# apache/paimon

Measured on NVIDIA H100. Metric: merged rows/sec at 16 runs x 40M rows, higher is better.
Workload: dtype int64

## Files before the change

### paimon_b200/csrc/parquet_decode.cu

```cuda
#include <algorithm>
#include <cstring>
#include <memory>
#include <stdexcept>

#include "device_utils.cuh"
#include "parquet_meta.h"
#include "inflate_device.cuh"
#include "scan_kernels.cuh"
#include "zstd_device.cuh"

namespace pg {

enum : int { ENC_PLAIN = 0, ENC_DICT = 1, ENC_DELTA_BP = 2, ENC_RLE_BOOL = 3 };

struct PqChunk {
    const uint8_t *base;
    int64_t avail;
    int64_t num_values;
    int64_t row0;
    int32_t col, run, file, codec;
    int32_t max_def, phys, phys_width;
    int32_t cast;
    int32_t n_pages, n_dicts;
    int64_t scratch_bytes;
// ... 794 lines not shown
                s_vs[warp][lane][c] = (int32_t)(p + bias);
                bias -= 4;
                p += 4 + len;
                if (++j == nnz) break;
            }
            if (bad || j == nnz) done = true;
        }
        __syncwarp();
        for (unsigned m = __ballot_sync(0xffffffffu, j > j0); m != 0; m &= m - 1) {
            const int i = __ffs(m) - 1;
            const int n = __shfl_sync(0xffffffffu, j - j0, i);
            int32_t *dst = (int32_t *)__shfl_sync(0xffffffffu, (unsigned long long)(uintptr_t)(vs + j0), i);
            if (lane < n) dst[lane] = s_vs[warp][i][lane];
        }
        WT_MARK(2);
        if (__all_sync(0xffffffffu, done)) break;
        const int cur = (int)(p / kWvChunk);
        const int first = max(next, cur);
        const int nreq = done ? 0 : max(0, min(min(cur, hist[0]) + kWvRing, n_chunks) - first);
        next = first + nreq;
        int incl = nreq;
#pragma unroll
        for (int d = 1; d < 32; d <<= 1) {
            const int y = __shfl_up_sync(0xffffffffu, incl, d);
            if (lane >= d) incl += y;
        }
        const int total = __shfl_sync(0xffffffffu, incl, 31);
        for (int r = 0; r < nreq; r++) {
            const int k = first + r;
            const uint32_t units = min(8u, (pend - (uint32_t)k * kWvChunk + 15) / 16);
            s_req_src[warp][incl - nreq + r] = a0 + (size_t)k * kWvChunk;
            s_req_dst[warp][incl - nreq + r] = (uint32_t)lane << 8 | (uint32_t)(k % kWvRing) << 4 | units;
        }
        __syncwarp();
        for (int e = lane >> 3; e < total; e += 4) {
            const uint32_t d = s_req_dst[warp][e], u = lane & 7;
            if (u < (d & 15)) {
                const int owner = (int)(d >> 8), unit = (int)(((d >> 4) & 15) * 8 + u);
                cp_async16(&rows[owner][(unit ^ (owner & 15)) << 4], s_req_src[warp][e] + 16 * u);
            }
        }
        cp_async_commit();
#pragma unroll
        for (int i = 0; i < kWvLead; i++) hist[i] = hist[i + 1];
        hist[kWvLead] = next;
        WT_MARK(0);
    }
    cp_async_wait<0>();
    WT_END(nnz);
    if (mine) {
        if (bad || (nnz > 0 && p != pend) || (nnz == 0 && slen != 0)) { pq_err(err, KERR_BAD_PAGE); pages[t].bad = 1; return; }
        vs[nnz] = (int32_t)(p + bias);
    }
}

constexpr int kExpThreads = 256;
constexpr int kPayIn = 8 * 1024, kPayOut = 7 * 1024;
constexpr int kPayBatches = 1023;


__device__ __forceinline__ uint64_t pq_load_unaligned(const uint8_t *p, int w) {
    if (w == 8) {
        const uintptr_t a = (uintptr_t)p;
        const uint64_t *q = (const uint64_t *)(a & ~(uintptr_t)7);
        const int sh = (int)(a & 7) * 8;
        const uint64_t lo = q[0];
        return sh ? (lo >> sh) | (q[1] << (64 - sh)) : lo;
    }
    const uintptr_t a = (uintptr_t)p;
    const uint32_t *q = (const uint32_t *)(a & ~(uintptr_t)3);
    const int sh = (int)(a & 3) * 8;
    const uint32_t lo = q[0];
    return sh ? (uint64_t)((lo >> sh) | (q[1] << (32 - sh))) : (uint64_t)lo;
}

template <bool kPlainStrings> struct PqPlainStage {
    int vs[2][kExpThreads + 4];
    int bnd[kPayBatches + 1];
    alignas(16) uint8_t in[2][kPayIn];
    alignas(16) uint8_t out[kPayOut];
};
template <> struct PqPlainStage<false> {};

template <bool kPlainStrings>
__global__ void __launch_bounds__(kExpThreads, 6)
k_pq_expand(const PqPage *pages, const PqPage *dicts, const PqChunk *chunks, const PqOut *outs, int n_cols,
            const int32_t *ids, const int32_t *vstart, const int32_t *dict_off, const int32_t *dict_len) {
    __shared__ uint32_t s_bits[kExpThreads];
    __shared__ int s_rank[kExpThreads];
    __shared__ int s_wlen[kExpThreads];
    __shared__ int s_ws[34];
    __shared__ PqPlainStage<kPlainStrings> stage;
    const PqPage pg = pages[blockIdx.x];
    if (pg.bad || pg.num_values == 0) return;
    const PqChunk ch = chunks[pg.chunk];
    if (kPlainStrings != (ch.phys == pq::T_BYTE_ARRAY && pg.enc == ENC_PLAIN)) return;
    const PqOut out = outs[ch.run * n_cols + ch.col];
    const int tid = threadIdx.x, lane = tid & 31, warp = tid >> 5;
    const int64_t row0 = pg.row0, row1 = pg.row0 + pg.num_values;
    const int64_t g0 = row0 & ~(int64_t)31;
    const int n_words = (int)((row1 - g0 + 31) >> 5);
    const uint8_t *values = pg.body + pg.values_off;
    const int pw = ch.phys_width;
    const bool varlen = ch.phys == pq::T_BYTE_ARRAY;
    const bool is_dict = pg.enc == ENC_DICT;
    const PqPage *dj = is_dict ? &dicts[ch.dict_base] : nullptr;
    const uint8_t *dbody = is_dict ? dj->body : nullptr;
    const int64_t ebase = is_dict ? dj->entry_base : 0;
    const int32_t *pids = ids + pg.ids_base;
    const int32_t *vs = vstart + pg.vs_base;
    uint8_t *payload = varlen ? (uint8_t *)out.data : nullptr;
    int carry_rank = 0;
    int64_t carry_bytes = pg.payload_base;
    for (int w0 = 0; w0 < n_words; w0 += kExpThreads) {
        const int jw = w0 + tid;
        uint32_t bits = 0;
        if (jw < n_words) {
            const int64_t wrow = g0 + 32 * (int64_t)jw;
            const int lo = wrow < row0 ? (int)(row0 - wrow) : 0;
            const int64_t hi = pq_min64(32, row1 - wrow);
            const uint32_t mask = (hi >= 32 ? 0xffffffffu : ((1u << hi) - 1)) & ~((1u << lo) - 1);
            bits = out.validity ? (out.validity[wrow >> 5] & mask) : mask;
        }
        int tot = 0;
        const int excl = block_scan_excl(__popc(bits), s_ws, &tot);
        s_bits[tid] = bits;
        s_rank[tid] = carry_rank + excl;
        __syncthreads();
        const int nw = min(kExpThreads, n_words - w0);
        if (varlen && is_dict) {
            for (int jj = warp; jj < nw; jj += kExpThreads / 32) {
                const uint32_t b = s_bits[jj];
                int len = 0;
                if ((b >> lane) & 1) len = dict_len[ebase + pids[s_rank[jj] + __popc(b & ((1u << lane) - 1))]];
#pragma unroll
                for (int d = 16; d > 0; d >>= 1) len += __shfl_xor_sync(0xffffffffu, len, d);
                if (lane == 0) s_wlen[jj] = len;
            }
            __syncthreads();
            int wtot = 0;
            const int wl = tid < nw ? s_wlen[tid] : 0;
            const int wex = block_scan_excl(wl, s_ws, &wtot);
            s_wlen[tid] = wex;
            __syncthreads();
            for (int jj = warp; jj < nw; jj += kExpThreads / 32) {
                const uint32_t b = s_bits[jj];
                const int64_t row = g0 + 32 * (int64_t)(w0 + jj) + lane;
                const bool inpage = row >= row0 && row < row1;
                int len = 0;
                const uint8_t *src = nullptr;
                if ((b >> lane) & 1) {
                    const int id = pids[s_rank[jj] + __popc(b & ((1u << lane) - 1))];
                    len = dict_len[ebase + id];
                    src = dbody + dict_off[ebase + id];
                }
                const int incl = warp_scan_incl(len);
                const int64_t off = carry_bytes + s_wlen[jj] + incl - len;
                if (inpage) out.offsets[row] = (int32_t)off;
                for (int r8 = 0; r8 < 32; r8 += 4) {
                    const int sl = r8 + (lane >> 3);
                    const int64_t o2 = __shfl_sync(0xffffffffu, off, sl);
                    const int l2 = __shfl_sync(0xffffffffu, len, sl);
                    const uint8_t *s2 = (const uint8_t *)__shfl_sync(0xffffffffu, (unsigned long long)(uintptr_t)src, sl);
                    for (int bb = lane & 7; bb < l2; bb += 8) payload[o2 + bb] = s2[bb];
                }
            }
            carry_bytes += wtot;
        } else {
            constexpr int kExpUnroll = 4, kStep = kExpThreads / 32;
            const int fmode = varlen ? 0 : pg.enc == ENC_RLE_BOOL ? 1 : ch.phys == pq::T_BOOLEAN ? 2 : is_dict ? 3 : 4;
            if (fmode == 4 && pw == 8 && out.out_width == 8 && ch.cast == 0) {
                constexpr int kPairUnroll = 2;
                const int half = lane >> 4, p0 = 2 * (lane & 15);
                const uintptr_t a0 = (uintptr_t)values;
                const int sh = (int)(a0 & 7) * 8;
                const uint64_t *q0 = (const uint64_t *)(a0 & ~(uintptr_t)7);
                uint64_t *od = (uint64_t *)out.data;
                for (int j0 = 2 * warp; j0 < nw; j0 += 2 * kStep * kPairUnroll) {
                    int64_t row[kPairUnroll];
// ... 100 lines not shown
        }
        carry_rank += tot;
        __syncthreads();
    }
    if (varlen) {
        if constexpr (kPlainStrings) {
            auto &s_vs = stage.vs;
            auto &s_bnd = stage.bnd;
            auto &s_in = stage.in;
            auto &s_out = stage.out;
            const int nnz = pg.nnz;
            const int64_t pb = pg.payload_base;
            const int nb = (nnz + kExpThreads - 1) / kExpThreads;
            const bool staged_page = nb <= kPayBatches;
            __syncthreads();
            if (staged_page) for (int i = tid; i <= nb; i += kExpThreads) s_bnd[i] = vs[min(i * kExpThreads, nnz)];
            __syncthreads();
            auto batch_src = [&](int b2) -> const uint8_t * { return values + ((int64_t)s_bnd[b2] - pb) + 4 * (int64_t)b2 * kExpThreads; };
            auto batch_fits = [&](int b2) -> bool {
                const int jn = min(kExpThreads, nnz - b2 * kExpThreads);
                const int out_len = s_bnd[b2 + 1] - s_bnd[b2];
                const int iskew = (int)((uintptr_t)batch_src(b2) & 15), oskew = (int)((uintptr_t)(payload + s_bnd[b2]) & 15);
                return iskew + out_len + 4 * jn <= kPayIn && oskew + out_len <= kPayOut;
            };
            auto prefetch = [&](int b2) {
                const int jn = min(kExpThreads, nnz - b2 * kExpThreads);
                int *dv = s_vs[b2 & 1];
                for (int i = tid; i <= jn; i += kExpThreads) cp_async4(dv + i, vs + b2 * kExpThreads + i);
                if (batch_fits(b2)) {
                    const uint8_t *src0 = batch_src(b2);
                    const int iskew = (int)((uintptr_t)src0 & 15);
                    const int n16 = (iskew + (s_bnd[b2 + 1] - s_bnd[b2]) + 4 * jn + 15) >> 4;
                    uint8_t *di = s_in[b2 & 1];
                    for (int i = tid; i < n16; i += kExpThreads) cp_async16(di + 16 * i, src0 - iskew + 16 * i);
                }
                cp_async_commit();
            };
            if (staged_page && nb > 0) prefetch(0);
            for (int b2 = 0; b2 < nb; b2++) {
                const int j0 = b2 * kExpThreads, jn = min(kExpThreads, nnz - j0);
                if (!staged_page) {
                    for (int t = tid >> 3; t < jn; t += kExpThreads / 8) {
                        const int st = vs[j0 + t], len = vs[j0 + t + 1] - st;
                        const uint8_t *src = values + ((int64_t)st - pb) + 4 * (int64_t)(j0 + t + 1);
                        for (int b3 = tid & 7; b3 < len; b3 += 8) payload[(int64_t)st + b3] = src[b3];
                    }
                    continue;
                }
                if (b2 + 1 < nb) { prefetch(b2 + 1); cp_async_wait<1>(); } else cp_async_wait<0>();
                __syncthreads();
                const int *cvs = s_vs[b2 & 1];
                const int out0 = s_bnd[b2], out_len = s_bnd[b2 + 1] - out0;
                if (batch_fits(b2)) {
                    const uint8_t *src0 = batch_src(b2);
                    const int iskew = (int)((uintptr_t)src0 & 15), oskew = (int)((uintptr_t)(payload + out0) & 15);
                    if (tid < jn) {
                        const int o = cvs[tid] - out0, len = cvs[tid + 1] - cvs[tid];
                        const uint8_t *sp = s_in[b2 & 1] + iskew + o + 4 * (tid + 1);
                        uint8_t *dp = s_out + oskew + o;
                        for (int b3 = 0; b3 < len; b3++) dp[b3] = sp[b3];
                    }
                    __syncthreads();
                    uint8_t *dst16 = payload + out0 - oskew;
                    const int end = oskew + out_len;
                    for (int c = tid; c * 16 < end; c += kExpThreads) {
                        const int c0 = c * 16;
                        if (c0 >= oskew && c0 + 16 <= end) *(uint4 *)(dst16 + c0) = *(const uint4 *)(s_out + c0);
                        else for (int b3 = max(c0, oskew); b3 < min(c0 + 16, end); b3++) dst16[b3] = s_out[b3];
                    }
                } else {
                    for (int t = tid >> 3; t < jn; t += kExpThreads / 8) {
                        const int st = cvs[t], len = cvs[t + 1] - st;
                        const uint8_t *src = values + ((int64_t)st - pb) + 4 * (int64_t)(j0 + t + 1);
                        for (int b3 = tid & 7; b3 < len; b3 += 8) payload[(int64_t)st + b3] = src[b3];
                    }
                }
                __syncthreads();
            }
        }
        if (pg.is_last && tid == 0) out.offsets[row1] = (int32_t)(pg.payload_base + pg.payload_bytes);
    }
}

__global__ void k_pq_zero_first_offset(const PqOut *outs, int n) {
    const int i = blockIdx.x * blockDim.x + threadIdx.x;
    if (i < n && outs[i].offsets) outs[i].offsets[0] = 0;
}


static int phys_cast(int pg_t, int phys) {
    switch (pg_t) {
        case PG_INT8: case PG_INT16: case PG_INT32: return phys == pq::T_INT32 ? 0 : -1;
        case PG_INT64: return phys == pq::T_INT64 ? 0 : (phys == pq::T_INT32 ? 1 : -1);
        case PG_FLOAT: return phys == pq::T_FLOAT ? 0 : -1;
        case PG_DOUBLE: return phys == pq::T_DOUBLE ? 0 : (phys == pq::T_FLOAT ? 2 : -1);
        case PG_BOOL: return phys == pq::T_BOOLEAN ? 0 : -1;
        case PG_STRING: case PG_BINARY: return phys == pq::T_BYTE_ARRAY ? 0 : -1;
        default: return -1;
    }
}
static int phys_width_of(int phys) {
    return phys == pq::T_INT32 || phys == pq::T_FLOAT ? 4 : (phys == pq::T_INT64 || phys == pq::T_DOUBLE ? 8 : 0);
}

static pg_status map_file_schema(RunBuilder &b, const pq::FileMetaData &m, int run) {
    if (m.schema.empty()) return fail(PG_ERR_FORMAT, "parquet: empty schema");
    const int nleaf = (int)m.schema.size() - 1;
    if (m.schema[0].num_children != nleaf)
        return fail(PG_ERR_UNSUPPORTED, "parquet: nested columns are not decoded on device (flat KeyValue file schemas are)");
    std::vector<std::string> cols(nleaf);
    for (int i = 1; i <= nleaf; i++) {
        if (m.schema[i].num_children != 0 || m.schema[i].repetition == pq::R_REPEATED)
            return fail(PG_ERR_UNSUPPORTED, "parquet: nested / repeated column " + m.schema[i].name);
        cols[i - 1] = m.schema[i].name;
    }
    { pg_status st = b.add_file(run, m.num_rows, cols); if (st) return st; }
    for (int c = 0; c < b.nc; c++) {
        const int fc = b.file_col.back()[c];
        if (fc < 0) continue;
        const pq::SchemaElement &e = m.schema[fc + 1];
        if (phys_cast(b.schema->field(c).type, e.type) < 0)
            return fail(PG_ERR_UNSUPPORTED, "parquet: column " + e.name + " has a physical type the device decoder "
                                            "does not map to the table type");
    }
    for (const pq::RowGroup &g : m.row_groups) {
        if ((int)g.columns.size() != nleaf) return fail(PG_ERR_FORMAT, "parquet: row group with a different column count");
        for (const pq::ColumnChunk &cc : g.columns)
            if (cc.codec != pq::C_UNCOMPRESSED && cc.codec != pq::C_SNAPPY && cc.codec != pq::C_ZSTD && cc.codec != pq::C_GZIP)
                return fail(PG_ERR_UNSUPPORTED, "parquet: compression codec " + std::to_string(cc.codec) +
                                                " is not decoded on device (UNCOMPRESSED, SNAPPY, ZSTD and GZIP are); write with "
                                                "'file.compression'='zstd' / 'snappy' / 'gzip' / 'none' or let the Java side decompress");
    }
    return PG_OK;
}

static pg_status kernel_error_status(int code) {
    switch (code) {
        case KERR_NONE: return PG_OK;
        case KERR_PQ_ENCODING:
            return fail(PG_ERR_UNSUPPORTED, "parquet: a page uses a value encoding the device decoder does not implement "
                                            "(PLAIN, dictionary, DELTA_BINARY_PACKED integers and RLE booleans are decoded)");
        case KERR_PQ_LEVELS:
            return fail(PG_ERR_UNSUPPORTED, "parquet: repetition levels / BIT_PACKED definition levels are not decoded on device");
        case KERR_PQ_NO_DICT: return fail(PG_ERR_FORMAT, "parquet: dictionary-encoded page without dictionary");
        case KERR_PQ_ROWS: return fail(PG_ERR_FORMAT, "parquet: page row counts do not add up");
        case KERR_PQ_HEADER: return fail(PG_ERR_FORMAT, "parquet: malformed or truncated page header");
        case KERR_PQ_DICT_ID: return fail(PG_ERR_FORMAT, "parquet: dictionary id outside the dictionary");
        case KERR_OFFSET_OVERFLOW: return fail(PG_ERR_INTERNAL, "parquet: a var-len column exceeds 2 GiB of payload");
        default: return fail(PG_ERR_FORMAT, "parquet: a page does not expand to its declared size");
    }
}

struct SectionFile {
    const uint8_t *bytes;
    int64_t size;
    int mem;
    int run;
    const pq::FileMetaData *meta;
};

static pg_status fetch_footers(const std::vector<SectionFile> &files, cudaStream_t sm, std::vector<pq::FileMetaData> &own_meta,
                               std::vector<const pq::FileMetaData *> &meta) {
    const int nf = (int)files.size();
    std::vector<int> need;
    for (int f = 0; f < nf; f++) {
        if (files[f].meta) meta[f] = files[f].meta;
        else if (files[f].mem == PG_MEM_DEVICE) need.push_back(f);
    }
    std::vector<uint8_t> tails(8 * need.size() + 8);
    SmallReads rb(sm);
    for (size_t i = 0; i < need.size(); i++) {
        pg_status rs = rb.add(tails.data() + 8 * i, files[need[i]].bytes + files[need[i]].size - 8, 8);
        if (rs) return rs;
    }
    if (!need.empty()) { pg_status rs = rb.finish(); if (rs) return rs; }
    std::vector<std::vector<uint8_t>> footers(need.size());
    try {
        for (size_t i = 0; i < need.size(); i++) {
            const int64_t flen = pq::footer_length(tails.data() + 8 * i);
            if (flen + 12 > files[need[i]].size) return fail(PG_ERR_FORMAT, "parquet: bad footer length");
            footers[i].resize((size_t)flen + 8);
            pg_status rs = rb.add(footers[i].data(), files[need[i]].bytes + files[need[i]].size - 8 - flen, (size_t)flen);
            if (rs) return rs;
        }
        if (!need.empty()) { pg_status rs = rb.finish(); if (rs) return rs; }
        for (size_t i = 0; i < need.size(); i++) {
            own_meta[need[i]] = pq::parse_footer_thrift(footers[i].data(), (int64_t)footers[i].size() - 8);
            meta[need[i]] = &own_meta[need[i]];
        }
        for (int f = 0; f < nf; f++)
            if (!meta[f]) {
                own_meta[f] = pq::parse_footer(files[f].bytes, files[f].size);
                meta[f] = &own_meta[f];
            }
    } catch (const std::exception &e) {
        return fail(PG_ERR_FORMAT, e.what());
    }
    return PG_OK;
}

struct ChunkTables {
    std::vector<PqChunk> chunks;
    std::vector<PqPair> pairs;
    bool any_snappy = false, any_delta = false, any_zstd = false;
    int64_t pair_rows = 0;
};

static pg_status build_chunk_tables(const Schema *s, const std::vector<SectionFile> &files,
                                    const std::vector<const uint8_t *> &d_file, const std::vector<const pq::FileMetaData *> &meta,
                                    const RunBuilder &b, ChunkTables &t) {
    const int nc = s->n_cols();
    const int n_runs = (int)b.run_rows.size();
    std::vector<std::vector<int>> run_files(n_runs);
    for (int f = 0; f < (int)files.size(); f++) run_files[files[f].run].push_back(f);
    for (int r = 0; r < n_runs; r++) {
        for (int c = 0; c < nc; c++) {
            if (!b.read[c]) continue;
            const int chunk0 = (int)t.chunks.size();
            for (int f : run_files[r]) {
                const pq::FileMetaData &m = *meta[f];
                const int fc = b.file_col[f][c];
                int64_t rg_row0 = 0;
                int64_t rows = 0;
                if (fc < 0) continue;
                for (const pq::RowGroup &g : m.row_groups) {
                    const pq::ColumnChunk &cc = g.columns[fc];
                    const int64_t start = cc.start();
                    if (cc.num_values != g.num_rows) return fail(PG_ERR_FORMAT, "parquet: page row counts do not add up");
                    if (cc.num_values == 0) continue;
                    if (start < 4 || start >= files[f].size) return fail(PG_ERR_FORMAT, "parquet: page offset out of range");
                    PqChunk ch;
                    memset(&ch, 0, sizeof(ch));
                    ch.base = d_file[f] + start;
                    ch.avail = std::min<int64_t>(cc.total_compressed_size > 0 ? cc.total_compressed_size : files[f].size,
                                                 files[f].size - start);
                    ch.num_values = cc.num_values;
                    ch.row0 = b.file_row0[f] + rg_row0;
                    ch.col = c; ch.run = r; ch.file = f; ch.codec = cc.codec;
                    ch.max_def = m.schema[fc + 1].repetition == pq::R_OPTIONAL ? 1 : 0;
                    ch.phys = cc.type;
                    ch.phys_width = phys_width_of(cc.type);
                    ch.cast = phys_cast(s->field(c).type, cc.type);
                    if (cc.type != m.schema[fc + 1].type) return fail(PG_ERR_FORMAT, "parquet: column chunk type differs from the schema");
                    if (cc.codec == pq::C_SNAPPY) t.any_snappy = true;
                    if (cc.codec == pq::C_ZSTD || cc.codec == pq::C_GZIP) t.any_zstd = true;
                    for (int32_t e : cc.encodings) if (e == pq::E_DELTA_BINARY_PACKED) t.any_delta = true;
                    if (cc.num_values > 0) t.chunks.push_back(ch);
                    rg_row0 += g.num_rows;
                    rows += g.num_rows;
                }
                if (rows != m.num_rows) return fail(PG_ERR_FORMAT, "parquet: row group row counts do not add up");
            }
            if (is_varlen(s->field(c).type)) {
                PqPair pr{r, c, chunk0, (int)t.chunks.size(), t.pair_rows, (int)t.pairs.size(), 0};
                t.pairs.push_back(pr);
                t.pair_rows += b.run_rows[r];
            }
        }
    }
    return PG_OK;
}

#ifdef PG_WALK_TIMING
static void walk_timing_dump() {
    static long long h[kWtSlots][8];
    cudaDeviceSynchronize();
    cudaMemcpyFromSymbol(h, g_walk_ts, sizeof(h));
    double acc[3] = {0, 0, 0}, steps = 0, vals = 0, steps_max = 0;
    long long g_lo = LLONG_MAX, g_hi = 0;
    int n = 0;
    for (int s = 0; s < kWtSlots; s++) {
        if (h[s][4] == 0) continue;
        n++;
        for (int k = 0; k < 3; k++) acc[k] += (double)h[s][k];
        steps += (double)h[s][3];
        steps_max = std::max(steps_max, (double)h[s][3]);
        vals += (double)h[s][4];
        g_lo = std::min(g_lo, h[s][5]);
        g_hi = std::max(g_hi, h[s][6]);
    }
    if (n == 0) return;
    const double tot = acc[0] + acc[1] + acc[2];
    fprintf(stderr, "[walk timing] %d warps: cycles per step issue %.0f wait %.0f walk %.0f (%.1f / %.1f / %.1f %%); "
                    "steps per warp %.1f (max %.0f), values per lane-step %.2f, span %.3f ms\n",
            n, acc[0] / steps, acc[1] / steps, acc[2] / steps, 100 * acc[0] / tot, 100 * acc[1] / tot, 100 * acc[2] / tot,
            steps / n, steps_max, vals / (32.0 * steps), (g_hi - g_lo) * 1e-6);
    int hist[10] = {0};
    double busy = 0;
    for (int s = 0; s < kWtSlots; s++) {
        if (h[s][4] == 0) continue;
        hist[std::min(9, (int)(10.0 * (h[s][5] - g_lo) / (double)(g_hi - g_lo + 1)))]++;
        busy += (double)(h[s][6] - h[s][5]);
    }
    fprintf(stderr, "[walk timing] warp start by tenth of the span:");
    for (int i = 0; i < 10; i++) fprintf(stderr, " %d", hist[i]);
    fprintf(stderr, "; mean warp lifetime %.3f ms\n", busy / n * 1e-6);
    static long long z[kWtSlots][8];
    cudaMemcpyToSymbol(g_walk_ts, z, sizeof(z));
}
#endif

static pg_status expand_pages(cudaStream_t sm, bool byte_arrays, PqPage *d_pages, int np, const PqPage *d_dicts,
                              const PqChunk *d_chunks, const PqOut *d_outs, int nc, const int32_t *d_ids, int32_t *d_vstart,
                              const int32_t *d_dict_off, const int32_t *d_dict_len, int32_t *d_err, int *launches) {
    if (!byte_arrays) {
        k_pq_expand<false><<<np, kExpThreads, 0, sm>>>(d_pages, d_dicts, d_chunks, d_outs, nc, d_ids, d_vstart,
                                                       d_dict_off, d_dict_len);
        (*launches)++;
        return PG_OK;
    }
    static thread_local cudaStream_t side = nullptr;
    static thread_local cudaEvent_t ev_fork = nullptr, ev_join = nullptr;
    if (!side) {
        int prio_lo = 0, prio_hi = 0;
        cudaDeviceGetStreamPriorityRange(&prio_lo, &prio_hi);
        PG_CUDA(cudaStreamCreateWithPriority(&side, cudaStreamNonBlocking, prio_hi));
        PG_CUDA(cudaEventCreateWithFlags(&ev_fork, cudaEventDisableTiming));
        PG_CUDA(cudaEventCreateWithFlags(&ev_join, cudaEventDisableTiming));
    }
    PG_CUDA(cudaEventRecord(ev_fork, sm));
    PG_CUDA(cudaStreamWaitEvent(side, ev_fork, 0));
    k_pq_walk_values<<<(np + kWvWarps * 32 - 1) / (kWvWarps * 32), kWvWarps * 32, 0, side>>>(
        d_pages, np, d_chunks, d_vstart, d_err);
    k_pq_expand<true><<<np, kExpThreads, 0, side>>>(d_pages, d_dicts, d_chunks, d_outs, nc, d_ids, d_vstart, d_dict_off,
                                                    d_dict_len);
    PG_CUDA(cudaEventRecord(ev_join, side));
    k_pq_expand<false><<<np, kExpThreads, 0, sm>>>(d_pages, d_dicts, d_chunks, d_outs, nc, d_ids, d_vstart, d_dict_off,
                                                   d_dict_len);
    PG_CUDA(cudaStreamWaitEvent(sm, ev_join, 0));
#ifdef PG_WALK_TIMING
    walk_timing_dump();
#endif
    *launches += 3;
    return PG_OK;
}

static pg_status decode_section(const std::shared_ptr<const Schema> &s, const std::vector<SectionFile> &files,
                                int n_runs, const char *const *names, const uint8_t *read_cols, uint64_t *out_runs,
                                pg_section_info *info) {
    const int nc = s->n_cols();
    const int nf = (int)files.size();
    cudaStream_t sm = copy_stream();
    Scratch scratch(sm);
    RunBuilder b(s, n_runs, scratch, "parquet");
    int launches = 0;
    SectionTimer tm;
    PG_CUDA(cudaEventCreate(&tm.e0));
    PG_CUDA(cudaEventCreate(&tm.e1));
    { pg_status st = b.read_columns(read_cols, names); if (st) return st; }

    std::vector<const uint8_t *> d_file(nf, nullptr);
    std::vector<pq::FileMetaData> own_meta(nf);
    std::vector<const pq::FileMetaData *> meta(nf, nullptr);
    int64_t file_bytes = 0, h2d = 0;
    PG_CUDA(cudaEventRecord(tm.e0, sm));
    for (int f = 0; f < nf; f++) {
        const SectionFile &sf = files[f];
        if (sf.size < 12) return fail(PG_ERR_FORMAT, "parquet: missing PAR1 magic (encrypted or not a Parquet file)");
        file_bytes += sf.size;
        if (sf.mem == PG_MEM_DEVICE) d_file[f] = sf.bytes;
        else {
            { pg_status st = file_image(scratch, sf.bytes, sf.size, "parquet", &d_file[f]); if (st) return st; }
            h2d += sf.size;
        }
    }
    { pg_status st = fetch_footers(files, sm, own_meta, meta); if (st) return st; }
    std::vector<uint8_t> any_optional(nc, 0);
    for (int f = 0; f < nf; f++) {
        pg_status st = map_file_schema(b, *meta[f], files[f].run);
        if (st) return st;
        for (int c = 0; c < nc; c++) {
            const int fc = b.file_col[f][c];
            if (fc == -1 || (fc >= 0 && meta[f]->schema[fc + 1].repetition == pq::R_OPTIONAL)) any_optional[c] = 1;
        }
    }
    { pg_status st = b.check_runs(); if (st) return st; }
    ChunkTables ct;
    { pg_status st = build_chunk_tables(s.get(), files, d_file, meta, b, ct); if (st) return st; }
    const int n_chunks = (int)ct.chunks.size(), n_pairs = (int)ct.pairs.size();

    { pg_status st = b.alloc(any_optional, b.missing); if (st) return st; }
    std::vector<PqOut> outs((size_t)n_runs * nc);
    auto fill_outs = [&] {
        for (size_t i = 0; i < outs.size(); i++) {
            const int t = s->field((int)(i % nc)).type;
            outs[i] = PqOut{b.out[i].data, b.out[i].offsets, b.out[i].validity, type_width(t), t == PG_BOOL};
        }
    };
    fill_outs();
    const bool any_empty = std::find(b.run_rows.begin(), b.run_rows.end(), 0) != b.run_rows.end();

    const size_t tb_chunks = align256(sizeof(PqChunk) * (size_t)std::max(n_chunks, 1));
    const size_t tb_outs = align256(sizeof(PqOut) * outs.size());
    const size_t tb_pairs = align256(sizeof(PqPair) * (size_t)std::max(n_pairs, 1));
    const size_t tb_tot = align256(sizeof(int64_t) * (size_t)(8 + n_pairs));
    unsigned char *tb = (unsigned char *)scratch.take(tb_chunks + tb_outs + tb_pairs + tb_tot + 256);
    if (!tb) return oom("parquet", "the chunk tables", tb_chunks + tb_outs + tb_pairs + tb_tot);
    PqChunk *d_chunks = (PqChunk *)tb;
    PqOut *d_outs = (PqOut *)(tb + tb_chunks);
    PqPair *d_pairs = (PqPair *)(tb + tb_chunks + tb_outs);
    int64_t *d_totals = (int64_t *)(tb + tb_chunks + tb_outs + tb_pairs);
    int32_t *d_err = (int32_t *)(d_totals + 6);
    PG_CUDA(cudaMemsetAsync(d_totals, 0, tb_tot, sm));
    if (n_chunks) { pg_status ts = small_h2d(d_chunks, ct.chunks.data(), sizeof(PqChunk) * n_chunks, sm); if (ts) return ts; }
    { pg_status ts = small_h2d(d_outs, outs.data(), sizeof(PqOut) * outs.size(), sm); if (ts) return ts; }
    if (n_pairs) { pg_status ts = small_h2d(d_pairs, ct.pairs.data(), sizeof(PqPair) * n_pairs, sm); if (ts) return ts; }
    int64_t h_tot[8] = {0, 0, 0, 0, 0, 0, 0, 0};
    if (n_chunks) {
        k_pq_walk<false><<<(n_chunks + 63) / 64, 64, 0, sm>>>(d_chunks, n_chunks, nullptr, nullptr, nullptr, d_err);
        k_pq_chunk_scan<<<1, kScanThreads, 0, sm>>>(d_chunks, n_chunks, d_totals);
        launches += 2;
// ... 3 lines not shown
            if (!rs) rs = rb.finish();
            if (rs) return rs;
        }
        const int herr = (int)(h_tot[6] & 0xffffffff);
        if (herr != KERR_NONE) return kernel_error_status(herr);
    }
    const int64_t n_pages = h_tot[0], n_dicts = h_tot[1], sc_bytes = h_tot[2], dict_entries = h_tot[3],
                  ids_entries = h_tot[4], page_bytes = h_tot[5];
    if (n_pages > 0x7fffffffLL) return fail(PG_ERR_UNSUPPORTED, "parquet: too many pages in one section");

    const size_t sb_pages = align256(sizeof(PqPage) * (size_t)std::max<int64_t>(n_pages, 1));
    const size_t sb_dicts = align256(sizeof(PqPage) * (size_t)std::max<int64_t>(n_dicts, 1));
    const size_t sb_sc = align256((size_t)sc_bytes + 64);
    const size_t sb_de = align256(4 * (size_t)(dict_entries + 1));
    const size_t sb_ids = align256(4 * (size_t)(ids_entries + 1));
    const size_t sb_vs = align256(4 * (size_t)(ct.pair_rows + n_pages + n_pairs + 2));
    int zs_ctas = 0;
    if (ct.any_zstd) {
        int dev = 0, sms = 132;
        cudaGetDevice(&dev);
        cudaDeviceGetAttribute(&sms, cudaDevAttrMultiProcessorCount, dev);
        zs_ctas = (int)std::min<int64_t>((int64_t)sms * 5, (n_pages + n_dicts + kZsWarps - 1) / kZsWarps);
    }
    const size_t sb_zs = align256((size_t)zs_ctas * kZsWarps * (size_t)(zs::kMaxBlock + 64));
    unsigned char *sbuf = (unsigned char *)scratch.take(sb_pages + sb_dicts + sb_sc + 2 * sb_de + sb_ids + sb_vs + sb_zs + 256);
    if (!sbuf) return oom("parquet", "the page table and scratch", sb_pages + sb_dicts + sb_sc + 2 * sb_de + sb_ids + sb_vs + sb_zs);
    PqPage *d_pages = (PqPage *)sbuf;
    PqPage *d_dicts = (PqPage *)(sbuf + sb_pages);
    uint8_t *d_sc = sbuf + sb_pages + sb_dicts;
    int32_t *d_dict_off = (int32_t *)(d_sc + sb_sc);
    int32_t *d_dict_len = (int32_t *)(d_sc + sb_sc + sb_de);
    int32_t *d_ids = (int32_t *)(d_sc + sb_sc + 2 * sb_de);
    int32_t *d_vstart = (int32_t *)(d_sc + sb_sc + 2 * sb_de + sb_ids);
    uint8_t *d_zs_lit = (uint8_t *)d_vstart + sb_vs;
    const int np = (int)n_pages, nd = (int)n_dicts;
    std::vector<int64_t> pair_tot(std::max(n_pairs, 1), 0);
    if (np > 0) {
        k_pq_walk<true><<<(n_chunks + 63) / 64, 64, 0, sm>>>(d_chunks, n_chunks, d_pages, d_dicts, d_sc, d_err);
        launches++;
        if (ct.any_snappy) {
            const int64_t th = (int64_t)(np + nd) * 32;
            k_pq_snappy<<<(unsigned)((th + 127) / 128), 128, 0, sm>>>(d_pages, np, d_dicts, nd, d_chunks, d_err);
            launches++;
        }
        if (ct.any_zstd && zs_ctas > 0) {
            k_pq_zstd<<<zs_ctas, kZsWarps * 32, 0, sm>>>(d_pages, np, d_dicts, nd, d_chunks, d_zs_lit, (int32_t *)(d_totals + 7), d_err);
            launches++;
        }
        if (ct.any_delta) {
            k_pq_delta<<<(unsigned)(((int64_t)np * 32 + 127) / 128), 128, 0, sm>>>(d_pages, np, d_chunks, d_err);
            launches++;
        }
        if (dict_entries > 0) {
            k_pq_walk_dicts<<<(nd + kWalkWarps - 1) / kWalkWarps, kWalkWarps * 32, 0, sm>>>(
                d_dicts, nd, d_chunks, d_dict_off, d_dict_len, d_err);
            launches++;
        }
        k_pq_levels<<<(unsigned)(((int64_t)np * 32 + 127) / 128), 128, 0, sm>>>(d_pages, np, d_dicts, d_chunks, d_outs, nc,
                                                                            d_ids, d_dict_len, d_err);
        launches++;
        if (n_pairs) {
            k_pq_scan_pages<<<(n_pairs * 32 + 127) / 128, 128, 0, sm>>>(d_pages, d_chunks, d_pairs, n_pairs, d_totals + 8, d_err);
            launches++;
            {
                SmallReads rb(sm);
                pg_status rs = rb.add(pair_tot.data(), d_totals + 8, sizeof(int64_t) * n_pairs);
                if (!rs) rs = rb.add(h_tot, d_totals, sizeof(int64_t) * 8);
                if (!rs) rs = rb.finish();
                if (rs) return rs;
            }
            const int herr = (int)(h_tot[6] & 0xffffffff);
            if (herr != KERR_NONE) return kernel_error_status(herr);
        }
    }

    if (n_pairs) {
        std::vector<int64_t> payload((size_t)n_runs * nc, 0);
        for (const PqPair &pr : ct.pairs) payload[(size_t)pr.run * nc + pr.col] = pair_tot[pr.idx];
        { pg_status st = b.alloc_payload(payload); if (st) return st; }
        fill_outs();
        { pg_status ts = small_h2d(d_outs, outs.data(), sizeof(PqOut) * outs.size(), sm); if (ts) return ts; }
    }
    if (np > 0) {
        pg_status st = expand_pages(sm, n_pairs > 0, d_pages, np, d_dicts, d_chunks, d_outs, nc, d_ids, d_vstart, d_dict_off,
                                    d_dict_len, d_err, &launches);
        if (st) return st;
    }
    if (any_empty && n_pairs) {
        k_pq_zero_first_offset<<<(n_runs * nc + 127) / 128, 128, 0, sm>>>(d_outs, n_runs * nc);
        launches++;
    }
    PG_CUDA(cudaEventRecord(tm.e1, sm));
    {
        SmallReads rb(sm);
        pg_status rs = rb.add(h_tot, d_totals, sizeof(int64_t) * 8);
        if (!rs) rs = rb.finish();
        if (rs) return rs;
    }
    PG_CUDA(cudaGetLastError());
    {
        const int herr = (int)(h_tot[6] & 0xffffffff);
        if (herr != KERR_NONE) return kernel_error_status(herr);
    }
    b.finish(out_runs, h2d, info);
    if (info) {
        info->file_bytes = file_bytes;
        info->page_bytes = page_bytes;
        info->n_files = nf;
        info->n_chunks = n_chunks;
        info->n_data_pages = np;
        info->n_dictionary_pages = nd;
        info->launches = launches;
        info->ms_decode = tm.ms();
    }
    return PG_OK;
}


struct PqReader {
    std::shared_ptr<const Schema> schema;
    pq::FileMetaData meta;
    std::vector<uint8_t> file;
    int64_t n_rows = 0;
    int n_data_pages = 0, n_dict_pages = 0;
    float ms_decode = 0;
    int launches = 0;
};

static Table<PqReader> g_pq(5);

static pg_status pq_open(uint64_t schema, const uint8_t *bytes, int64_t size, uint64_t *out) {
    std::shared_ptr<Schema> s = g_schemas.get(schema);
    if (!s || !bytes || !out) return fail(PG_ERR_INVALID, "bad schema handle or null argument");
    auto rd = std::make_unique<PqReader>();
    rd->schema = s;
    try {
        rd->meta = pq::parse_footer(bytes, size);
    } catch (const std::exception &e) {
        return fail(PG_ERR_FORMAT, e.what());
    }
    const pq::FileMetaData &m = rd->meta;
    Scratch scratch(nullptr);
    RunBuilder b(s, 1, scratch, "parquet");
    pg_status st = map_file_schema(b, m, 0);
    if (st) return st;
    const int nc = s->n_cols();
    rd->n_rows = m.num_rows;
    int64_t row0 = 0;
    for (const pq::RowGroup &g : m.row_groups) {
        for (int c = 0; c < nc; c++) {
            const pq::ColumnChunk &cc = g.columns[c];
            const int max_def = m.schema[c + 1].repetition == pq::R_OPTIONAL ? 1 : 0;
            int64_t pos = cc.start(), vals = 0;
            bool have_dict = false;
            while (vals < cc.num_values) {
                if (pos < 4 || pos >= size) return fail(PG_ERR_FORMAT, "parquet: page offset out of range");
                PqHeader h;
                if (!pq_parse_header(bytes + pos, bytes + size, h)) return fail(PG_ERR_FORMAT, "parquet: malformed or truncated page header");
                const int64_t body = pos + h.hdr;
                if (h.comp < 0 || body + h.comp > size) return fail(PG_ERR_FORMAT, "parquet: truncated page");
                if (h.type == pq::P_DICTIONARY) {
                    if (h.enc != pq::E_PLAIN && h.enc != pq::E_PLAIN_DICTIONARY)
                        return fail(PG_ERR_UNSUPPORTED, "parquet: dictionary page encoding");
                    have_dict = true;
                    rd->n_dict_pages++;
                } else if (h.type == pq::P_DATA || h.type == pq::P_DATA_V2) {
                    const bool is_dict = h.enc == pq::E_PLAIN_DICTIONARY || h.enc == pq::E_RLE_DICTIONARY;
                    const bool is_delta = h.enc == pq::E_DELTA_BINARY_PACKED && (cc.type == pq::T_INT32 || cc.type == pq::T_INT64);
// ... 202 lines not shown
```

### profiles/decode_kernels.py

```python
import argparse
import collections
import json
import os
import subprocess
import sys
import tempfile

ROOT = os.path.dirname(os.path.dirname(os.path.abspath(__file__)))
sys.path.insert(0, ROOT)
os.environ.setdefault("PG_RUN_CACHE_BYTES", str(64 << 30))


def gpu_identity(index):
    try:
        out = subprocess.run(["nvidia-smi", "-i", str(index), "--query-gpu=name,power.limit,clocks.max.sm",
                              "--format=csv,noheader"], capture_output=True, text=True, timeout=30).stdout.strip()
        name, power, clock = [x.strip() for x in out.split(",")]
        return {"name": name, "power_limit": power, "clocks_max_sm": clock}
    except Exception as e:
        import torch
        return {"name": torch.cuda.get_device_name(index), "power_limit": None, "error": repr(e)[:200]}


def decode_windows(kernels):
    wins, cur = [], []
    for k in kernels:
        if "k_pq_walk<false>" in k["name"] and cur:
            wins.append(cur)
            cur = []
        cur.append(k)
    if cur:
        wins.append(cur)
    return wins


def short(name):
    n = name.split("(")[0]
    return n.replace("pg::", "").replace("void ", "")


def main():
    ap = argparse.ArgumentParser()
    ap.add_argument("--rows", type=int, default=None, help="total input rows (default: the bench's C3 size)")
    ap.add_argument("--reps", type=int, default=3)
    ap.add_argument("--warmup", type=int, default=2)
    ap.add_argument("--out", default=os.path.join(tempfile.gettempdir(), "decode_kernels"))
    args = ap.parse_args()

    import torch
    from torch.profiler import ProfilerActivity, profile

    import bench
    from paimon_b200 import _native as N
    from paimon_b200.format import read_section

    dev = torch.device("cuda", 0)
    torch.cuda.set_device(dev)
    w = bench.WORKLOADS["c3"]
    rows = args.rows or w["rows"]
    schema = bench.make_schema("c3")
    lib = N.init(0)
    _, images, _, _ = bench.device_parquet_files("c3", schema, rows, dev, 100, lib)
    files = [(img, r) for r, img in enumerate(images)]

    def decode():
        readers, info = read_section(schema, files, w["n_runs"], 0)
        for r in readers:
            r.close()
        return info

    for _ in range(args.warmup):
        decode()
    torch.cuda.synchronize()
    infos = []
    with profile(activities=[ProfilerActivity.CUDA]) as prof:
        for _ in range(args.reps):
            infos.append(decode())
        torch.cuda.synchronize()
    os.makedirs(args.out, exist_ok=True)
    trace = os.path.join(args.out, "trace.pt.trace.json")
    prof.export_chrome_trace(trace)
    with open(trace) as f:
        ev = json.load(f)["traceEvents"]
    kernels = sorted(({"name": e["name"], "ts": float(e["ts"]), "dur": float(e["dur"]),
                       "stream": e.get("args", {}).get("stream")}
                      for e in ev if e.get("cat") == "kernel" and "k_pq" in e.get("name", "")),
                     key=lambda k: k["ts"])
    wins = decode_windows(kernels)
    n = len(wins)

    per = collections.defaultdict(lambda: {"launches": 0, "ms": 0.0})
    for k in kernels:
        key = (short(k["name"]), k["stream"])
        per[key]["launches"] += 1
        per[key]["ms"] += k["dur"] / 1e3
    main_stream = wins[0][0]["stream"] if wins else None
    table = [{"kernel": name, "stream": s, "side": s != main_stream, "launches_per_decode": v["launches"] / n,
              "ms_per_decode": v["ms"] / n} for (name, s), v in per.items()]
    table.sort(key=lambda r: -r["ms_per_decode"])

    spans = []
    for win in wins:
        t0 = win[0]["ts"]
        t1 = max(k["ts"] + k["dur"] for k in win)
        side = [k for k in win if k["stream"] != main_stream]
        mains = [k for k in win if k["stream"] == main_stream]
        exp_main = [k for k in mains if "k_pq_expand" in k["name"]]
        gaps = [(b["ts"] - (a["ts"] + a["dur"])) / 1e3 for a, b in zip(mains, mains[1:])]
        spans.append({
            "stage_ms": (t1 - t0) / 1e3,
            "side_fork_to_join_ms": ((max(k["ts"] + k["dur"] for k in side) - min(k["ts"] for k in side)) / 1e3
                                     if side else 0.0),
            "main_expand_ms": sum(k["dur"] for k in exp_main) / 1e3,
            "main_stream_gaps_ms": [round(g, 3) for g in gaps],
            "main_stream_idle_ms": sum(max(g, 0.0) for g in gaps),
        })
    summary = {
        "gpu": gpu_identity(0),
        "rows": rows,
        "decodes": n,
        "pages": int(infos[-1].n_data_pages),
        "launches": int(infos[-1].launches),
        "ms_decode_events": [round(i.ms_decode, 3) for i in infos],
        "kernels": table,
        "per_decode": spans,
    }
    with open(os.path.join(args.out, "summary.json"), "w") as f:
        json.dump(summary, f, indent=1)
    with open(os.path.join(args.out, "kernels.csv"), "w") as f:
        f.write("kernel,stream,side,launches_per_decode,ms_per_decode\n")
        for r in table:
            f.write(f"{r['kernel']},{r['stream']},{int(r['side'])},{r['launches_per_decode']:g},{r['ms_per_decode']:.3f}\n")

    print(json.dumps(summary["gpu"]), f"rows={rows} pages={summary['pages']} launches={summary['launches']}")
    print("ms_decode (CUDA events):", summary["ms_decode_events"])
    print(f"{'kernel':<28}{'stream':>8}{'side':>6}{'launches':>10}{'ms':>10}")
    for r in table:
        print(f"{r['kernel']:<28}{str(r['stream']):>8}{int(r['side']):>6}{r['launches_per_decode']:>10g}"
              f"{r['ms_per_decode']:>10.3f}")
    for i, s in enumerate(spans):
        print(f"decode {i}: stage {s['stage_ms']:.3f} ms, side fork->join {s['side_fork_to_join_ms']:.3f} ms, "
              f"main expand {s['main_expand_ms']:.3f} ms, main-stream idle {s['main_stream_idle_ms']:.3f} ms "
              f"(gaps {s['main_stream_gaps_ms']})")


if __name__ == "__main__":
    main()
```

Before: 905.0 million.

## Add dedicated TMA-pipelined expand kernel for plain fixed-width parquet pages

Adds k_pq_expand_fixed, which handles PLAIN 4/8-byte pages. It streams page values into a shared-memory ring using bulk async copies tracked by mbarriers, computes validity ranks per span with a block scan, and writes int64 pairs as 16-byte stores. The general expand kernel now skips these pages and is launched only when dictionary pages or other types are present. The aim is to cut the latency-bound global loads and per-word overhead of the generic expand path. The cost is more code complexity and the ring/mbarrier synchronisation. The profiling script also gains bandwidth reporting.

```diff
diff --git a/paimon_b200/csrc/parquet_decode.cu b/paimon_b200/csrc/parquet_decode.cu
--- a/paimon_b200/csrc/parquet_decode.cu
+++ b/paimon_b200/csrc/parquet_decode.cu
@@ -900,6 +900,10 @@
 };
 template <> struct PqPlainStage<false> {};
 
+__device__ __forceinline__ bool pq_fixed_plain(const PqPage &pg, const PqChunk &ch) {
+    return (ch.phys_width == 4 || ch.phys_width == 8) && pg.enc != ENC_DICT && pg.enc != ENC_RLE_BOOL;
+}
+
 template <bool kPlainStrings>
 __global__ void __launch_bounds__(kExpThreads, 6)
 k_pq_expand(const PqPage *pages, const PqPage *dicts, const PqChunk *chunks, const PqOut *outs, int n_cols,
@@ -913,6 +917,7 @@
     if (pg.bad || pg.num_values == 0) return;
     const PqChunk ch = chunks[pg.chunk];
     if (kPlainStrings != (ch.phys == pq::T_BYTE_ARRAY && pg.enc == ENC_PLAIN)) return;
+    if (!kPlainStrings && pq_fixed_plain(pg, ch)) return;
     const PqOut out = outs[ch.run * n_cols + ch.col];
     const int tid = threadIdx.x, lane = tid & 31, warp = tid >> 5;
     const int64_t row0 = pg.row0, row1 = pg.row0 + pg.num_values;
@@ -1179,6 +1184,151 @@
     }
 }
 
+constexpr int kFxThreads = 256, kFxSpanPer = 3, kFxSpanWords = kFxSpanPer * kFxThreads;
+constexpr int kFxWinWords = 32, kFxWarpWords = kFxWinWords / (kFxThreads / 32);
+constexpr int kFxChunk = 2048, kFxChunks = 8, kFxRing = kFxChunk * kFxChunks;
+static_assert((kFxRing & (kFxRing - 1)) == 0 && kFxWinWords * 32 * 8 + 8 <= (kFxChunks - 3) * kFxChunk &&
+              kFxWarpWords % 2 == 0, "ring shape");
+
+__global__ void __launch_bounds__(kFxThreads, 6)
+k_pq_expand_fixed(const PqPage *pages, const PqChunk *chunks, const PqOut *outs, int n_cols) {
+    __shared__ alignas(16) uint8_t s_ring[kFxRing];
+    __shared__ uint32_t s_bits[kFxSpanWords];
+    __shared__ int s_rank[kFxSpanWords + 1];
+    __shared__ int s_ws[34];
+    __shared__ uint64_t s_bar[kFxChunks];
+    const PqPage pg = pages[blockIdx.x];
+    if (pg.bad || pg.num_values == 0) return;
+    const PqChunk ch = chunks[pg.chunk];
+    if (!pq_fixed_plain(pg, ch)) return;
+    const PqOut out = outs[ch.run * n_cols + ch.col];
+    const int tid = threadIdx.x, lane = tid & 31, warp = tid >> 5;
+    const int64_t row0 = pg.row0, row1 = pg.row0 + pg.num_values;
+    const int64_t g0 = row0 & ~(int64_t)31;
+    const int n_words = (int)((row1 - g0 + 31) >> 5);
+    const int pw = ch.phys_width;
+    const uint8_t *values = pg.body + pg.values_off;
+    const int skew = (int)((uintptr_t)values & 15);
+    const uint8_t *a0 = values - skew;
+    const int n_bytes = skew + pg.nnz * pw;
+    const int n_chunks = pg.nnz > 0 ? (n_bytes + kFxChunk - 1) / kFxChunk : 0;
+    const int copy_end = (n_bytes + 15) & ~15;
+    int issued = 0;
+    auto issue_below = [&](int c_end) {
+        c_end = min(c_end, n_chunks);
+        if (issued < c_end) asm volatile("fence.proxy.async.shared::cta;" ::: "memory");
+        for (; issued < c_end; issued++) {
+            const int s = issued % kFxChunks;
+            const uint32_t bytes = (uint32_t)min(kFxChunk, copy_end - issued * kFxChunk);
+            mbar_arrive_expect_tx(&s_bar[s], bytes);
+            bulk_g2s(s_ring + s * kFxChunk, a0 + (int64_t)issued * kFxChunk, bytes, &s_bar[s]);
+        }
+    };
+    if (tid == 0) {
+        for (int s = 0; s < kFxChunks; s++) mbar_init(&s_bar[s], 1);
+        mbar_fence_init();
+        issue_below(kFxChunks);
+    }
+    const bool opt = out.validity != nullptr;
+    auto word_mask = [&](int j) -> uint32_t {
+        const int64_t wrow = g0 + 32 * (int64_t)j;
+        const int lo = wrow < row0 ? (int)(row0 - wrow) : 0;
+        const int64_t hi = pq_min64(32, row1 - wrow);
+        return (hi >= 32 ? 0xffffffffu : ((1u << hi) - 1)) & ~((1u << lo) - 1);
+    };
+    const int sh8 = (skew & 7) * 8, sh4 = (skew & 3) * 8;
+    auto value_at = [&](int r) -> uint64_t {
+        if (pw == 8) {
+            const int a = (skew & ~7) + 8 * r;
+            const uint64_t lo = *(const uint64_t *)(s_ring + (a & (kFxRing - 1)));
+            if (!sh8) return lo;
+            const uint64_t hi = *(const uint64_t *)(s_ring + ((a + 8) & (kFxRing - 1)));
+            return (lo >> sh8) | (hi << (64 - sh8));
+        }
+        const int a = (skew & ~3) + 4 * r;
+        const uint32_t lo = *(const uint32_t *)(s_ring + (a & (kFxRing - 1)));
+        const uint32_t hi = sh4 ? *(const uint32_t *)(s_ring + ((a + 4) & (kFxRing - 1))) : 0u;
+        return (uint64_t)__funnelshift_r(lo, hi, sh4);
+    };
+    const bool pair_path = pw == 8 && out.out_width == 8 && ch.cast == 0;
+    uint64_t *od = (uint64_t *)out.data;
+    int carry = 0;
+    __syncthreads();
+    for (int s0 = 0; s0 < n_words; s0 += kFxSpanWords) {
+        const int ns = min(kFxSpanWords, n_words - s0);
+        if (opt) {
+            uint32_t b[kFxSpanPer];
+            int c[kFxSpanPer], sum = 0;
+#pragma unroll
+            for (int i = 0; i < kFxSpanPer; i++) {
+                const int j = kFxSpanPer * tid + i;
+                b[i] = j < ns ? out.validity[(g0 >> 5) + s0 + j] & word_mask(s0 + j) : 0u;
+                c[i] = sum;
+                sum += __popc(b[i]);
+            }
+            int tot = 0;
+            const int excl = carry + block_scan_excl(sum, s_ws, &tot);
+#pragma unroll
+            for (int i = 0; i < kFxSpanPer; i++) {
+                s_bits[kFxSpanPer * tid + i] = b[i];
+                s_rank[kFxSpanPer * tid + i] = excl + c[i];
+            }
+            carry += tot;
+            if (tid == 0) s_rank[kFxSpanWords] = carry;
+            __syncthreads();
+        }
+        auto word_bits = [&](int j) -> uint32_t { return opt ? s_bits[j] : word_mask(s0 + j); };
+        auto word_rank = [&](int j) -> int {
+            if (opt) return s_rank[j];
+            const int64_t wrow = g0 + 32 * (int64_t)(s0 + j);
+            return (int)(wrow < row0 ? 0 : pq_min64(wrow - row0, row1 - row0));
+        };
+        for (int w0 = 0; w0 < ns; w0 += kFxWinWords) {
+            const int nw = min(kFxWinWords, ns - w0);
+            const int r_lo = word_rank(w0), r_hi = word_rank(w0 + nw);
+            if (r_hi > r_lo) {
+                const int c_lo = (skew + r_lo * pw) / kFxChunk, c_hi = (skew + r_hi * pw - 1) / kFxChunk;
+                for (int c = c_lo; c <= c_hi; c++) mbar_wait(&s_bar[c % kFxChunks], (uint32_t)(c / kFxChunks) & 1);
+            }
+            if (pair_path) {
+                const int half = lane >> 4, p0 = 2 * (lane & 15);
+#pragma unroll
+                for (int k = 0; k < kFxWarpWords / 2; k++) {
+                    const int jj = w0 + kFxWarpWords * warp + 2 * k + half;
+                    if (jj >= w0 + nw) continue;
+                    const uint32_t b = word_bits(jj);
+                    const int rk = word_rank(jj) + __popc(b & ((1u << p0) - 1));
+                    const bool v0 = (b >> p0) & 1, v1 = (b >> (p0 + 1)) & 1;
+                    const int64_t row = g0 + 32 * (int64_t)(s0 + jj) + p0;
+                    const bool in0 = row >= row0 && row < row1, in1 = row + 1 >= row0 && row + 1 < row1;
+                    const uint64_t x0 = v0 ? value_at(rk) : 0, x1 = v1 ? value_at(rk + v0) : 0;
+                    if (in0 && in1) *(ulonglong2 *)(od + row) = make_ulonglong2(x0, x1);
+                    else if (in0) od[row] = x0;
+                    else if (in1) od[row + 1] = x1;
+                }
+            } else {
+#pragma unroll
+                for (int k = 0; k < kFxWarpWords; k++) {
+                    const int jj = w0 + kFxWarpWords * warp + k;
+                    if (jj >= w0 + nw) continue;
+                    const uint32_t b = word_bits(jj);
+                    const int64_t row = g0 + 32 * (int64_t)(s0 + jj) + lane;
+                    if (row < row0 || row >= row1) continue;
+                    uint64_t x = 0;
+                    if ((b >> lane) & 1) {
+                        x = value_at(word_rank(jj) + __popc(b & ((1u << lane) - 1)));
+                        if (ch.cast == 1) x = (uint64_t)(int64_t)(int32_t)(uint32_t)x;
+                        else if (ch.cast == 2) x = (uint64_t)__double_as_longlong((double)__uint_as_float((uint32_t)x));
+                    }
+                    store_fixed(out.data, out.out_width, row, x);
+                }
+            }
+            __syncthreads();
+            if (tid == 0) issue_below((skew + r_hi * pw) / kFxChunk + kFxChunks);
+        }
+    }
+}
+
 __global__ void k_pq_zero_first_offset(const PqOut *outs, int n) {
     const int i = blockIdx.x * blockDim.x + threadIdx.x;
     if (i < n && outs[i].offsets) outs[i].offsets[0] = 0;
@@ -1300,6 +1450,7 @@
     std::vector<PqChunk> chunks;
     std::vector<PqPair> pairs;
     bool any_snappy = false, any_delta = false, any_zstd = false;
+    bool any_other_type = false;
     int64_t pair_rows = 0;
 };
 
@@ -1342,6 +1493,7 @@
                     if (cc.codec == pq::C_SNAPPY) t.any_snappy = true;
                     if (cc.codec == pq::C_ZSTD || cc.codec == pq::C_GZIP) t.any_zstd = true;
                     for (int32_t e : cc.encodings) if (e == pq::E_DELTA_BINARY_PACKED) t.any_delta = true;
+                    if (ch.phys_width == 0 && cc.type != pq::T_BYTE_ARRAY) t.any_other_type = true;
                     if (cc.num_values > 0) t.chunks.push_back(ch);
                     rg_row0 += g.num_rows;
                     rows += g.num_rows;
@@ -1397,13 +1549,17 @@
 }
 #endif
 
-static pg_status expand_pages(cudaStream_t sm, bool byte_arrays, PqPage *d_pages, int np, const PqPage *d_dicts,
+static pg_status expand_pages(cudaStream_t sm, bool byte_arrays, bool general, PqPage *d_pages, int np, const PqPage *d_dicts,
                               const PqChunk *d_chunks, const PqOut *d_outs, int nc, const int32_t *d_ids, int32_t *d_vstart,
                               const int32_t *d_dict_off, const int32_t *d_dict_len, int32_t *d_err, int *launches) {
     if (!byte_arrays) {
-        k_pq_expand<false><<<np, kExpThreads, 0, sm>>>(d_pages, d_dicts, d_chunks, d_outs, nc, d_ids, d_vstart,
-                                                       d_dict_off, d_dict_len);
+        k_pq_expand_fixed<<<np, kFxThreads, 0, sm>>>(d_pages, d_chunks, d_outs, nc);
         (*launches)++;
+        if (general) {
+            k_pq_expand<false><<<np, kExpThreads, 0, sm>>>(d_pages, d_dicts, d_chunks, d_outs, nc, d_ids, d_vstart,
+                                                           d_dict_off, d_dict_len);
+            (*launches)++;
+        }
         return PG_OK;
     }
     static thread_local cudaStream_t side = nullptr;
@@ -1422,8 +1578,12 @@
     k_pq_expand<true><<<np, kExpThreads, 0, side>>>(d_pages, d_dicts, d_chunks, d_outs, nc, d_ids, d_vstart, d_dict_off,
                                                     d_dict_len);
     PG_CUDA(cudaEventRecord(ev_join, side));
-    k_pq_expand<false><<<np, kExpThreads, 0, sm>>>(d_pages, d_dicts, d_chunks, d_outs, nc, d_ids, d_vstart, d_dict_off,
-                                                   d_dict_len);
+    k_pq_expand_fixed<<<np, kFxThreads, 0, sm>>>(d_pages, d_chunks, d_outs, nc);
+    if (general) {
+        k_pq_expand<false><<<np, kExpThreads, 0, sm>>>(d_pages, d_dicts, d_chunks, d_outs, nc, d_ids, d_vstart,
+                                                       d_dict_off, d_dict_len);
+        (*launches)++;
+    }
     PG_CUDA(cudaStreamWaitEvent(sm, ev_join, 0));
 #ifdef PG_WALK_TIMING
     walk_timing_dump();
@@ -1593,8 +1753,8 @@
         { pg_status ts = small_h2d(d_outs, outs.data(), sizeof(PqOut) * outs.size(), sm); if (ts) return ts; }
     }
     if (np > 0) {
-        pg_status st = expand_pages(sm, n_pairs > 0, d_pages, np, d_dicts, d_chunks, d_outs, nc, d_ids, d_vstart, d_dict_off,
-                                    d_dict_len, d_err, &launches);
+        pg_status st = expand_pages(sm, n_pairs > 0, nd > 0 || ct.any_other_type, d_pages, np, d_dicts, d_chunks, d_outs, nc,
+                                    d_ids, d_vstart, d_dict_off, d_dict_len, d_err, &launches);
         if (st) return st;
     }
     if (any_empty && n_pairs) {
diff --git a/profiles/decode_kernels.py b/profiles/decode_kernels.py
--- a/profiles/decode_kernels.py
+++ b/profiles/decode_kernels.py
@@ -39,6 +39,41 @@
     return n.replace("pg::", "").replace("void ", "")
 
 
+def fixed_width_bytes(bench, schema, rows, dev, seed):
+    import torch
+    from paimon_b200.types import PhysicalType, is_varlen
+    file_width = {PhysicalType.INT8: 4, PhysicalType.INT16: 4, PhysicalType.INT32: 4, PhysicalType.INT64: 8,
+                  PhysicalType.FLOAT: 4, PhysicalType.DOUBLE: 8}
+    out_width = {PhysicalType.INT8: 1, PhysicalType.INT16: 2, PhysicalType.INT32: 4, PhysicalType.INT64: 8,
+                 PhysicalType.FLOAT: 4, PhysicalType.DOUBLE: 8}
+    w = bench.WORKLOADS["c3"]
+    n_runs = w["n_runs"]
+    per_run = rows // n_runs
+    key_space = max(rows // 2, per_run)
+    table = torch.tensor([bin(i).count("1") for i in range(256)], device=dev, dtype=torch.int64)
+    enc = dec = 0
+    for r in range(n_runs):
+        cols, keep, _, _, _ = bench.gen_device_run(schema, r, per_run, key_space, w["null_prob"], seed, dev,
+                                                   w.get("delete_prob", 0.0))
+        by_ptr = {t.data_ptr(): t for t in keep}
+        for f, c in zip(schema.file_fields(), cols):
+            t = f.physical
+            if is_varlen(t):
+                continue
+            nnz = per_run
+            if c.validity:
+                v = by_ptr[c.validity][:per_run // 8]
+                nnz = int(table[v.long()].sum().item())
+                tail = per_run % 8
+                if tail:
+                    nnz += bin(int(by_ptr[c.validity][per_run // 8].item()) & ((1 << tail) - 1)).count("1")
+            enc += nnz * file_width[t]
+            dec += per_run * out_width[t]
+        del cols, keep, by_ptr
+    torch.cuda.synchronize()
+    return enc, dec
+
+
 def main():
     ap = argparse.ArgumentParser()
     ap.add_argument("--rows", type=int, default=None, help="total input rows (default: the bench's C3 size)")
@@ -62,6 +97,7 @@
     lib = N.init(0)
     _, images, _, _ = bench.device_parquet_files("c3", schema, rows, dev, 100, lib)
     files = [(img, r) for r, img in enumerate(images)]
+    fx_enc, fx_dec = fixed_width_bytes(bench, schema, rows, dev, 100)
 
     def decode():
         readers, info = read_section(schema, files, w["n_runs"], 0)
@@ -107,11 +143,13 @@
         mains = [k for k in win if k["stream"] == main_stream]
         exp_main = [k for k in mains if "k_pq_expand" in k["name"]]
         gaps = [(b["ts"] - (a["ts"] + a["dur"])) / 1e3 for a, b in zip(mains, mains[1:])]
+        exp_ms = sum(k["dur"] for k in exp_main) / 1e3
         spans.append({
             "stage_ms": (t1 - t0) / 1e3,
             "side_fork_to_join_ms": ((max(k["ts"] + k["dur"] for k in side) - min(k["ts"] for k in side)) / 1e3
                                      if side else 0.0),
-            "main_expand_ms": sum(k["dur"] for k in exp_main) / 1e3,
+            "main_expand_ms": exp_ms,
+            "main_expand_gbs": (fx_enc + fx_dec) / (exp_ms * 1e-3) / 1e9 if exp_ms > 0 else 0.0,
             "main_stream_gaps_ms": [round(g, 3) for g in gaps],
             "main_stream_idle_ms": sum(max(g, 0.0) for g in gaps),
         })
@@ -122,6 +160,7 @@
         "pages": int(infos[-1].n_data_pages),
         "launches": int(infos[-1].launches),
         "ms_decode_events": [round(i.ms_decode, 3) for i in infos],
+        "main_expand_bytes": {"encoded_fixed_width_values": fx_enc, "decoded_fixed_width": fx_dec},
         "kernels": table,
         "per_decode": spans,
     }
@@ -134,13 +173,15 @@
 
     print(json.dumps(summary["gpu"]), f"rows={rows} pages={summary['pages']} launches={summary['launches']}")
     print("ms_decode (CUDA events):", summary["ms_decode_events"])
+    print(f"main-stream expansion bytes: {fx_enc / 1e9:.3f} GB fixed-width values read + {fx_dec / 1e9:.3f} GB "
+          f"fixed-width columns written")
     print(f"{'kernel':<28}{'stream':>8}{'side':>6}{'launches':>10}{'ms':>10}")
     for r in table:
         print(f"{r['kernel']:<28}{str(r['stream']):>8}{int(r['side']):>6}{r['launches_per_decode']:>10g}"
               f"{r['ms_per_decode']:>10.3f}")
     for i, s in enumerate(spans):
         print(f"decode {i}: stage {s['stage_ms']:.3f} ms, side fork->join {s['side_fork_to_join_ms']:.3f} ms, "
-              f"main expand {s['main_expand_ms']:.3f} ms, main-stream idle {s['main_stream_idle_ms']:.3f} ms "
+              f"main expand {s['main_expand_ms']:.3f} ms ({s['main_expand_gbs']:.0f} GB/s), main-stream idle {s['main_stream_idle_ms']:.3f} ms "
               f"(gaps {s['main_stream_gaps_ms']})")
 
 
```

Result: faster. 929.0 million (median of 6 runs) (+2.7%).
